# IRFM/librir

Hardware: NVIDIA B200
Metric: frames/s at 640x512 u16 (full per-frame pipeline: bad-pixel correct + gaussian + translate + pre-coder) (higher is better)
Workload: dtype u16

## Files before the change

include/librir_b200.h:

```cpp
#ifndef LIBRIR_B200_H
#define LIBRIR_B200_H

#include <stddef.h>
#include <stdint.h>

#ifdef __cplusplus
extern "C" {
#endif

#define RIRB_API __attribute__((visibility("default")))


RIRB_API int translate(int type, void* src, void* dst, int w, int h, float dx, float dy, void* background,
                       const char* strategy);

RIRB_API int gaussian_filter(float* src, float* dst, int w, int h, float sigma);

RIRB_API int find_median_pixel(unsigned short* pixels, int size, float percent);
RIRB_API int find_median_pixel_mask(unsigned short* pixels, unsigned char* mask, int size, float percent);

RIRB_API int bad_pixels_create(unsigned short* first_image, int width, int height);
RIRB_API int bad_pixels_correct(int handle, unsigned short* in, unsigned short* out);
RIRB_API void bad_pixels_destroy(int handle);

// ... 59 lines not shown
RIRB_API int rirb_decode_movie(const unsigned char* lo, const unsigned char* hi, long long nframes, int w, int h, int gop,
                               int delta, long long first_frame, unsigned short* movie);
RIRB_API int rirb_key_frames(long long nframes, int gop, unsigned char* key);

RIRB_API int rirb_lossy_open(int w, int h, int stop_lossy_height, int low_error, int high_error, double std_factor,
                             int running_average, int subtract_min, int remove_bad_pixels);
RIRB_API int rirb_lossy_add_images(int handle, const unsigned short* frames, long long nframes, unsigned short* out, int* errors);
RIRB_API int rirb_lossy_set_parameter(int handle, const char* key, const char* value);
RIRB_API void rirb_lossy_close(int handle);
RIRB_API int rirb_lossy_get_min(int handle, int* min_value);

RIRB_API int rirb_process_movie_host(int handle, const unsigned short* frames, long long nframes, int w, int h, float sigma,
                                     const float* dx, const float* dy, const char* strategy, unsigned int background, int gop,
                                     int delta, long long first_frame, unsigned char* lo, unsigned char* hi, float* smoothed);


RIRB_API int rirb_movie_stats(const unsigned short* pixels, size_t n, unsigned int* minmax, unsigned long long* hist,
                              int accumulate);
RIRB_API int rirb_hist_quantile(const unsigned long long* hist, long long count, float percent);
RIRB_API int rirb_get_background(const unsigned short* pixels, int size);


RIRB_API int rirb_attrs_open_file(const char* filename);
RIRB_API int rirb_attrs_open_from_memory(const void* ptr, long long size);
RIRB_API void rirb_attrs_close(int handle);
RIRB_API void rirb_attrs_discard(int handle);
RIRB_API void rirb_attrs_abandon(int handle);
RIRB_API int rirb_attrs_flush(int handle);
RIRB_API int rirb_attrs_image_count(int handle);
RIRB_API int rirb_attrs_global_attribute_count(int handle);
// ... 58 lines not shown
```

librir_b200/_lib.py:

```python
from __future__ import annotations

import ctypes as ct
import glob
import os

_HERE = os.path.dirname(os.path.abspath(__file__))
LIB_DIR = os.path.join(_HERE, "libs")


def lib_path() -> str:
    found = sorted(glob.glob(os.path.join(LIB_DIR, "*signal_processing*.so")))
    if not found:
        raise ImportError(
            "librir_b200: libs/libsignal_processing_b200.so is not built "
            "(run `python -c 'import __graft_entry__ as g; g.build()'` or `make -C librir_b200/csrc`)"
        )
    return found[0]


_vp, _i, _ll, _f, _sz = ct.c_void_p, ct.c_int, ct.c_longlong, ct.c_float, ct.c_size_t

SIGNATURES = {
    "translate": (_i, [_i, _vp, _vp, _i, _i, _f, _f, _vp, ct.c_char_p]),
    "gaussian_filter": (_i, [_vp, _vp, _i, _i, _f]),
# ... 29 lines not shown
    "rirb_split_yuv444": (_i, [_vp, _vp, _i, _i, _vp, _vp, _vp, _i, _i, _i]),
    "rirb_merge_yuv444": (_i, [_vp, _vp, _vp, _i, _i, _i, _i, _i, _vp, _vp]),
    "rirb_split_yuv420": (_i, [_vp, _vp, _i, _i, _vp, _i, _vp, _i]),
    "rirb_merge_yuv420": (_i, [_vp, _i, _vp, _i, _i, _i, _vp, _vp]),
    "rirb_precode_movie": (_i, [_vp, _ll, _i, _i, _i, _i, _ll, _vp, _vp]),
    "rirb_precode_movie_stats": (_i, [_vp, _ll, _i, _i, _i, _i, _ll, _vp, _vp, _vp, _vp, _i]),
    "rirb_decode_movie": (_i, [_vp, _vp, _ll, _i, _i, _i, _i, _ll, _vp]),
    "rirb_key_frames": (_i, [_ll, _i, _vp]),
    "rirb_lossy_open": (_i, [_i, _i, _i, _i, _i, ct.c_double, _i, _i, _i]),
    "rirb_lossy_add_images": (_i, [_i, _vp, _ll, _vp, _vp]),
    "rirb_lossy_close": (None, [_i]),
    "rirb_lossy_get_min": (_i, [_i, _vp]),
    "rirb_release_thread_resources": (None, []),
    "rirb_lossy_set_parameter": (_i, [_i, ct.c_char_p, ct.c_char_p]),
    "rirb_process_movie_host": (_i, [_i, _vp, _ll, _i, _i, _f, _vp, _vp, ct.c_char_p, ct.c_uint, _i, _i, _ll, _vp, _vp, _vp]),
    "rirb_movie_stats": (_i, [_vp, _sz, _vp, _vp, _i]),
    "rirb_hist_quantile": (_i, [_vp, _ll, _f]),
    "rirb_get_background": (_i, [_vp, _i]),
    "rirb_attrs_open_file": (_i, [ct.c_char_p]),
    "rirb_attrs_open_from_memory": (_i, [_vp, _ll]),
    "rirb_attrs_close": (None, [_i]),
    "rirb_attrs_discard": (None, [_i]),
    "rirb_attrs_abandon": (None, [_i]),
    "rirb_attrs_flush": (_i, [_i]),
    "rirb_attrs_image_count": (_i, [_i]),
    "rirb_attrs_global_attribute_count": (_i, [_i]),
    "rirb_attrs_global_attribute_name": (_i, [_i, _i, _vp, _vp]),
    "rirb_attrs_global_attribute_value": (_i, [_i, _i, _vp, _vp]),
    "rirb_attrs_frame_attribute_count": (_i, [_i, _i]),
    "rirb_attrs_frame_attribute_name": (_i, [_i, _i, _i, _vp, _vp]),
# ... 79 lines not shown
```

librir_b200/csrc/capi.cu:

```cuda
#include <dlfcn.h>
#include <math.h>
#include <stdarg.h>
#include <stdlib.h>
#include <string.h>

#include <map>
#include <memory>
#include <mutex>
#include <vector>

#include "../../include/librir_b200.h"
#include "common.cuh"
#include "kernels.h"

namespace rirb {

std::atomic<long long> g_launches{0};

struct ThreadState {
    char err[512] = {0};
    cudaStream_t stream = 0;
    static constexpr int SLOTS = 12;
    void* dev[SLOTS] = {};
    size_t cap[SLOTS] = {};
// ... 1482 lines not shown
        if (!ok(cudaMemcpyAsync(lo + a * fpx, d_lo, fpx * m, cudaMemcpyDefault, st), "download of the low-byte planes") ||
            !ok(cudaMemcpyAsync(hi + a * fpx, d_hi, fpx * m, cudaMemcpyDefault, st), "download of the high-byte planes") ||
            (smoothed && !ok(cudaMemcpyAsync(smoothed + a * fpx, d_sm, fpx * 4 * m, cudaMemcpyDefault, st), "download of the smoothed frames")))
            break;
    }
    for (int q = 0; q < HP_SLOTS; ++q) {
        cudaError_t e = cudaStreamSynchronize(hp.slot[q].stream);
        if (e != cudaSuccess && rc == 0) {
            set_error("process_movie_host: %s", cudaGetErrorString(e));
            rc = -1;
        }
    }
    return rc;
}

void rirb_release_thread_resources(void)
{
    if (tls.stream) (void)cudaStreamSynchronize(tls.stream);
    g_host_pipe.release();
    for (int d = 0; d < PIN_MAX_DEVICES; ++d) pin_rings[d].release();
    tls.release();
}

int rirb_movie_stats(const unsigned short* pixels, size_t n, unsigned int* minmax, unsigned long long* hist, int accumulate)
{
    if (!pixels || !minmax) {
        set_error("movie_stats: bad arguments");
        return -1;
    }
    RIRB_REQUIRE_DEVICE();
// ... 126 lines not shown
```

librir_b200/csrc/kernels.h:

```cpp
#pragma once
#include <cuda_runtime.h>
#include <stddef.h>

#include <initializer_list>

namespace rirb {

typedef unsigned short u16;
typedef unsigned char u8;

enum { STRAT_NOBORDER = 0, STRAT_BACKGROUND = 1, STRAT_WRAP = 2, STRAT_NEAREST = 3 };

int launch_hist_frame(const u16* img, size_t n, unsigned* hist65536, cudaStream_t st);
int launch_bp_detect(const u16* img, int w, int h, double std_factor, unsigned gthr, u8* mask, cudaStream_t st);
constexpr int BP_SPAN = 16384;
int launch_bp_correct(const u16* in, u16* out, const int* xy_dev, const int* span_off_dev, int w, int h, int clamp_value,
                      long long nframes, size_t frame_stride, cudaStream_t st);
int launch_bp_correct_inplace(u16* img, const int* xy_dev, int count, int w, int h, int clamp_value, long long nframes,
                              size_t frame_stride, cudaStream_t st);
int launch_loader_bp(u16* img, const int* xy_dev, const u8* mask, int count, int w, int h, long long nframes,
                     size_t frame_stride, cudaStream_t st);

int launch_loader_merge(const u8* lo, const u8* hi, u16* out, int w, int h, int hb, long long nframes, size_t frame_stride,
                        int min_t, int min_t_height, const int* xy_dev, const int* span_off_dev, const int* nbr_dev,
                        cudaStream_t st);

int launch_loader_add_min(u16* frames, int w, int t_rows, long long nframes, size_t frame_stride, int min_t, cudaStream_t st);
int launch_loader_fused(const u8* lo, const u8* hi, u16* out, int w, int h_full, int hb, long long nframes, int min_t, int t_rows,
                        const int* xy_dev, const int* nbr_dev, const int* row_off_dev, const u8* mask_dev, const float* dxs,
                        const float* dys, cudaStream_t st);

int launch_translate(int type, const void* src, void* dst, int w, int h, long long nframes, const float* dxs, const float* dys,
                     float dx0, float dy0, int strategy, const void* background_host, cudaStream_t st);
int launch_translate_u16(const u16* src, u16* dst, int w, int h, long long nframes, size_t src_stride, size_t dst_stride,
                         const float* dxs, const float* dys, float dx0, float dy0, int strategy, unsigned background, bool motion,
                         cudaStream_t st);

constexpr int GAUSS_MAX_RADIUS = 64;
struct GaussTaps {
    int radius;
    float k[2 * GAUSS_MAX_RADIUS + 1];
};
int gaussian_taps_host(float sigma, GaussTaps* taps);
int launch_gaussian_f32(const float* src, float* dst, int w, int h, long long nframes, const GaussTaps& taps, cudaStream_t st);
int launch_gaussian_u16(const u16* src, float* dst, int w, int h, long long nframes, const GaussTaps& taps, cudaStream_t st);
int launch_gaussian_u16_region(const u16* src, size_t src_row, size_t src_frame, float* dst, int w, int h, long long nframes,
                               const GaussTaps& taps, cudaStream_t st);
int launch_gaussian_f32_region(const float* src, size_t src_row, size_t src_frame, float* dst, int w, int h, long long nframes,
                               const GaussTaps& taps, cudaStream_t st);
int launch_gaussian_bp_u16(const u16* raw, u16* corrected, float* dst, int w, int h, long long nframes, const GaussTaps& taps,
                           const int* xy_dev, const int* row_off_dev, int clamp_value, cudaStream_t st);
// ... 44 lines not shown
inline int refuse_pageable(const char* what, std::initializer_list<Operand> ops)
{
    for (const Operand& o : ops)
        if (o.p && operand_memory_type(o.p) == cudaMemoryTypeUnregistered) {
            set_error("%s: %s is pageable host memory; pass device, managed or pinned memory", what, o.name);
            return -1;
        }
    return 0;
}

int launch_split_planes(const u16* img, const u8* it, int w, int h, u8* y_plane, u8* u_plane, u8* v_plane, int ls_y, int ls_u,
                        int ls_v, cudaStream_t st);
int launch_merge_planes(const u8* y_plane, const u8* u_plane, const u8* v_plane, int ls_y, int ls_u, int ls_v, int w, int h,
                        u16* img, u8* it, cudaStream_t st);
int launch_precode_movie(const u16* mov, long long nframes, int w, int h, int gop, int delta, long long first_frame, u8* lo,
                         u8* hi, cudaStream_t st);
int launch_precode_movie_stats(const u16* mov, long long nframes, int w, int h, int gop, int delta, long long first_frame, u8* lo,
                               u8* hi, unsigned* minmax, unsigned long long* hist, cudaStream_t st);
int launch_decode_movie(const u8* lo, const u8* hi, long long nframes, int w, int h, int gop, int delta, long long first_frame,
                        u16* mov, cudaStream_t st);

size_t zcoder_scratch_bytes(long long n, long long bytes_each, long long segment);
long long zcoder_frame_bound(long long bytes_each, long long segment);
int launch_zstd_encode(const u8* src, long long n, long long bytes_each, long long segment, u8* dst, long long dst_stride,
                       int rec_head, long long* sizes, long long** frame_offsets, void* scratch, cudaStream_t st);
size_t zcoder_lz_scratch_bytes(long long n, long long bytes_each, long long segment);
int launch_zstd_encode_lz(const u8* src, long long n, long long bytes_each, long long segment, u8* dst, long long dst_stride,
                          int rec_head, long long* sizes, long long** frame_offsets, void* scratch, cudaStream_t st);
size_t zdecoder_scratch_bytes(long long n, long long cap);
int zdecoder_frame_plain(const u8* f, long long size, long long cap);
int launch_zstd_decode(const u8* src, const long long* offsets, const unsigned* sizes, long long n, u8* dst, long long dst_stride,
                       long long cap, long long* status, void* scratch, cudaStream_t st);

// ... 23 lines not shown
```

librir_b200/csrc/precode.cu:

```cuda
#include "common.cuh"
#include "hist.cuh"
#include "kernels.h"

namespace rirb {

struct LoHi {
    uint4 lo, hi;
};

__device__ __forceinline__ LoHi split16(const U32x8& p)
{
    LoHi r;
    r.lo.x = __byte_perm(p.v[0], p.v[1], 0x6420);
    r.lo.y = __byte_perm(p.v[2], p.v[3], 0x6420);
    r.lo.z = __byte_perm(p.v[4], p.v[5], 0x6420);
    r.lo.w = __byte_perm(p.v[6], p.v[7], 0x6420);
    r.hi.x = __byte_perm(p.v[0], p.v[1], 0x7531);
    r.hi.y = __byte_perm(p.v[2], p.v[3], 0x7531);
    r.hi.z = __byte_perm(p.v[4], p.v[5], 0x7531);
    r.hi.w = __byte_perm(p.v[6], p.v[7], 0x7531);
    return r;
}

__device__ __forceinline__ U32x8 merge16(const uint4& lo, const uint4& hi)
// ... 73 lines not shown
__device__ __forceinline__ U32x8 sub16(const U32x8& a, const U32x8& b)
{
    U32x8 r;
#pragma unroll
    for (int i = 0; i < 8; ++i) r.v[i] = __vsub2(a.v[i], b.v[i]);
    return r;
}
__device__ __forceinline__ U32x8 add16(const U32x8& a, const U32x8& b)
{
    U32x8 r;
#pragma unroll
    for (int i = 0; i < 8; ++i) r.v[i] = __vadd2(a.v[i], b.v[i]);
    return r;
}

__global__ void __launch_bounds__(PC_THREADS)
delta_split_kernel(const u16* __restrict__ mov, u8* __restrict__ lo, u8* __restrict__ hi, size_t vec_per_frame, long long nframes,
                   int gop)
{
    const size_t i = (size_t)blockIdx.x * PC_THREADS + threadIdx.x;
    if (i >= vec_per_frame) return;
    const long long t0 = (long long)blockIdx.y * gop;
    const long long t1 = min(nframes, t0 + gop);
    U32x8 prev;
#pragma unroll
    for (int k = 0; k < 8; ++k) prev.v[k] = 0;
    for (long long t = t0; t < t1; t += PC_UNROLL) {
        U32x8 cur[PC_UNROLL];
#pragma unroll
        for (int k = 0; k < PC_UNROLL; ++k)
            if (t + k < t1) cur[k] = ld_stream256(mov + ((size_t)(t + k) * vec_per_frame + i) * 16);
#pragma unroll
        for (int k = 0; k < PC_UNROLL; ++k)
            if (t + k < t1) {
                LoHi r = split16(sub16(cur[k], prev));
                prev = cur[k];
                const size_t o = (size_t)(t + k) * vec_per_frame + i;
                st_stream(reinterpret_cast<uint4*>(lo) + o, r.lo);
                st_stream(reinterpret_cast<uint4*>(hi) + o, r.hi);
            }
    }
// ... 17 lines not shown
            if (t + k < t1) {
                const size_t o = (size_t)(t + k) * vec_per_frame + i;
                l[k] = ld_stream(reinterpret_cast<const uint4*>(lo) + o);
                h[k] = ld_stream(reinterpret_cast<const uint4*>(hi) + o);
            }
#pragma unroll
        for (int k = 0; k < PC_UNROLL; ++k)
            if (t + k < t1) {
                prev = add16(merge16(l[k], h[k]), prev);
                st_stream256(mov + ((size_t)(t + k) * vec_per_frame + i) * 16, prev);
            }
    }
}

__global__ void delta_split_scalar_kernel(const u16* __restrict__ mov, u8* __restrict__ lo, u8* __restrict__ hi, size_t npx,
                                          long long nframes, int gop)
{
    const size_t i = (size_t)blockIdx.x * blockDim.x + threadIdx.x;
    if (i >= npx) return;
    const long long t0 = (long long)blockIdx.y * gop;
    const long long t1 = min(nframes, t0 + gop);
    unsigned prev = 0;
    for (long long t = t0; t < t1; ++t) {
        unsigned cur = mov[(size_t)t * npx + i];
        unsigned r = (cur - prev) & 0xFFFFu;
        prev = cur;
        lo[(size_t)t * npx + i] = (u8)(r & 0xFF);
        hi[(size_t)t * npx + i] = (u8)(r >> 8);
    }
}
__global__ void delta_merge_scalar_kernel(const u8* __restrict__ lo, const u8* __restrict__ hi, u16* __restrict__ mov, size_t npx,
                                          long long nframes, int gop)
{
    const size_t i = (size_t)blockIdx.x * blockDim.x + threadIdx.x;
    if (i >= npx) return;
    const long long t0 = (long long)blockIdx.y * gop;
    const long long t1 = min(nframes, t0 + gop);
// ... 5 lines not shown
    }
}

constexpr long long MAX_GOPS_PER_LAUNCH = 65535;

static bool movie_vectorizable(const void* mov, const void* lo, const void* hi, size_t npx)
{
    return (npx % 16 == 0) && aligned32(mov) && aligned16(lo) && aligned16(hi);
}

constexpr int PS_THREADS = 1024;

template <bool DELTA>
__global__ void __launch_bounds__(PS_THREADS, 1)
split_stats_kernel(const u16* __restrict__ mov, u8* __restrict__ lo, u8* __restrict__ hi, size_t vec_per_frame, long long nframes,
                   int gop, unsigned* __restrict__ minmax, unsigned long long* __restrict__ hist)
{
    extern __shared__ unsigned sh[];
    for (unsigned i = threadIdx.x; i < HIST_SMEM_BINS; i += PS_THREADS) sh[i] = 0;
    __syncthreads();
    const long long ngop = (nframes + gop - 1) / gop;
    const long long blocks = (long long)((vec_per_frame + PS_THREADS - 1) / PS_THREADS);
    unsigned lo2 = 0xFFFFFFFFu, hi2 = 0u;
    for (long long item = blockIdx.x; item < blocks * ngop; item += gridDim.x) {
        const long long g = item / blocks;
        const size_t i = (size_t)(item - g * blocks) * PS_THREADS + threadIdx.x;
        if (i >= vec_per_frame) continue;
        const long long t0 = g * gop, t1 = min(nframes, t0 + gop);
        U32x8 prev;
#pragma unroll
        for (int k = 0; k < 8; ++k) prev.v[k] = 0;
        for (long long t = t0; t < t1; t += PC_UNROLL) {
            U32x8 cur[PC_UNROLL];
#pragma unroll
            for (int k = 0; k < PC_UNROLL; ++k)
                if (t + k < t1) cur[k] = ld_stream256(mov + ((size_t)(t + k) * vec_per_frame + i) * 16);
#pragma unroll
            for (int k = 0; k < PC_UNROLL; ++k)
                if (t + k < t1) {
                    const LoHi r = split16(DELTA ? sub16(cur[k], prev) : cur[k]);
                    if (DELTA) prev = cur[k];
                    const size_t o = (size_t)(t + k) * vec_per_frame + i;
                    st_stream(reinterpret_cast<uint4*>(lo) + o, r.lo);
                    st_stream(reinterpret_cast<uint4*>(hi) + o, r.hi);
#pragma unroll
                    for (int q = 0; q < 8; ++q) {
                        const unsigned w2 = cur[k].v[q];
                        lo2 = __vminu2(lo2, w2);
                        hi2 = __vmaxu2(hi2, w2);
                        count_px(w2 & 0xFFFFu, sh, hist);
                        count_px(w2 >> 16, sh, hist);
                    }
                }
        }
    }
    hist_flush(min(lo2 & 0xFFFFu, lo2 >> 16), max(hi2 & 0xFFFFu, hi2 >> 16), sh, minmax, hist, true);
}

int launch_precode_movie_stats(const u16* mov, long long nframes, int w, int h, int gop, int delta, long long first_frame, u8* lo,
                               u8* hi, unsigned* minmax, unsigned long long* hist, cudaStream_t st)
{
    if (nframes <= 0 || w <= 0 || h <= 0) return 0;
    const size_t npx = (size_t)w * h;
    if (gop < 1) gop = 1;
    if (!movie_vectorizable(mov, lo, hi, npx) || !hist || !minmax) return 1;
    if (delta && first_frame % gop != 0) {
        set_error("precode: with delta on, a shard must start on a key frame (first_frame %lld, GOP %d)", first_frame, gop);
        return -1;
    }
    const size_t vpf = npx / 16;
    const size_t smem = HIST_SMEM_BINS * sizeof(unsigned);
    const long long items = ceil_div((long long)vpf, PS_THREADS) * ceil_div(nframes, gop);
    const unsigned grid = (unsigned)min((long long)sm_count(), items);
    if (delta) {
        RIRB_SMEM_ATTR(split_stats_kernel<true>, smem);
        RIRB_LAUNCH(split_stats_kernel<true>, grid, PS_THREADS, smem, st, mov, lo, hi, vpf, nframes, gop, minmax, hist);
    } else {
        RIRB_SMEM_ATTR(split_stats_kernel<false>, smem);
        RIRB_LAUNCH(split_stats_kernel<false>, grid, PS_THREADS, smem, st, mov, lo, hi, vpf, nframes, gop, minmax, hist);
    }
    return 0;
}

int launch_precode_movie(const u16* mov, long long nframes, int w, int h, int gop, int delta, long long first_frame, u8* lo,
                         u8* hi, cudaStream_t st)
{
    if (nframes <= 0 || w <= 0 || h <= 0) return 0;
    const size_t npx = (size_t)w * h;
    if (gop < 1) gop = 1;
    if (!delta) {
        const size_t n = npx * (size_t)nframes;
        size_t done = 0;
        if (aligned32(mov) && aligned16(lo) && aligned16(hi) && n >= 16) {
            const size_t nvec = n / 16;
            RIRB_LAUNCH(split_flat_kernel, (unsigned)ceil_div((long long)nvec, PC_THREADS * PC_UNROLL), PC_THREADS, 0, st, mov, lo,
                        hi, nvec);
            done = nvec * 16;
        }
        if (done < n)
            RIRB_LAUNCH(split_scalar_kernel, (unsigned)ceil_div((long long)(n - done), 256), 256, 0, st, mov, lo, hi, done, n);
        return 0;
    }
    if (first_frame % gop != 0) {
        set_error("precode: with delta on, a shard must start on a key frame (first_frame %lld, GOP %d)", first_frame, gop);
        return -1;
    }
    const bool vec = movie_vectorizable(mov, lo, hi, npx);
    const long long span = (long long)MAX_GOPS_PER_LAUNCH * gop;
    for (long long f0 = 0; f0 < nframes; f0 += span) {
        const long long n = min(nframes - f0, span);
        const size_t off = (size_t)f0 * npx;
        const unsigned ngop = (unsigned)ceil_div(n, gop);
        if (vec) {
            const size_t vpf = npx / 16;
            dim3 grid((unsigned)ceil_div((long long)vpf, PC_THREADS), ngop);
            RIRB_LAUNCH(delta_split_kernel, grid, PC_THREADS, 0, st, mov + off, lo + off, hi + off, vpf, n, gop);
        } else {
            dim3 grid((unsigned)ceil_div((long long)npx, 256), ngop);
            RIRB_LAUNCH(delta_split_scalar_kernel, grid, 256, 0, st, mov + off, lo + off, hi + off, npx, n, gop);
        }
    }
    return 0;
}

int launch_decode_movie(const u8* lo, const u8* hi, long long nframes, int w, int h, int gop, int delta, long long first_frame,
                        u16* mov, cudaStream_t st)
{
    if (nframes <= 0 || w <= 0 || h <= 0) return 0;
    const size_t npx = (size_t)w * h;
    if (gop < 1) gop = 1;
    if (!delta) {
        const size_t n = npx * (size_t)nframes;
        size_t done = 0;
        if (aligned32(mov) && aligned16(lo) && aligned16(hi) && n >= 16) {
// ... 75 lines not shown
```

librir_b200/csrc/translate.cu:

```cuda
#include <stdlib.h>

#include "common.cuh"
#include "kernels.h"
#include "sort9.cuh"
#include "tma.cuh"

namespace rirb {

template <typename T> struct Pix {
    __device__ static __forceinline__ double to_double(T v) { return (double)v; }
    __device__ static __forceinline__ T from_double(double v) { return (T)v; }
};
struct BoolPix {
    u8 v;
};
template <> struct Pix<BoolPix> {
    __device__ static __forceinline__ double to_double(BoolPix b) { return b.v ? 1.0 : 0.0; }
    __device__ static __forceinline__ BoolPix from_double(double v) { return BoolPix{(u8)(v != 0.0)}; }
};

__device__ __forceinline__ unsigned long long f2size(float v) { return (unsigned long long)(long long)v; }
__device__ __forceinline__ unsigned long long wrap_idx(unsigned long long v, unsigned long long n) { return (v + n) % n; }

__device__ __forceinline__ double blend4(double p1, double p2, double p3, double p4, double u, double v)
// ... 711 lines not shown
        unpack9<XOFF>(lds128(srow), lds128(srow + 16), pb);
        if (clamp_rt) pb[8] = pb[7];
        unsigned A, B;
        asm volatile("ld.shared.v2.u32 {%0,%1}, [%2];" : "=r"(A), "=r"(B) : "r"(rab + k * (int)sizeof(RowAB)));
        if (B != ROW_SLOW) blend_rows<XOFF, MOTION>(pb, pt, A, B, ca, cb, magic, orow);
        orow += w;
#pragma unroll
        for (int j = 0; j < 9; ++j) pt[j] = pb[j];
    }
}

template <bool MOTION>
__global__ void __launch_bounds__(TW_THREADS, 5)
translate_u16_rows_kernel(const __grid_constant__ CUtensorMap tmap, const u16* __restrict__ src, u16* __restrict__ dst, int w, int h,
                          size_t src_stride, size_t dst_stride, const float* __restrict__ dxs, const float* __restrict__ dys,
                          float dx0, float dy0, int strategy, unsigned background, int tiles_y, const int* __restrict__ order)
{
    extern __shared__ __align__(128) unsigned char smem_raw[];
    __shared__ __align__(8) unsigned long long bar[TT_STAGES];
    __shared__ __align__(8) RowAB rowab[3][TT_H];
    __shared__ unsigned done[TT_STAGES];
    __shared__ EdgeTable edge_tab[2];
    const int f = order ? order[blockIdx.y] : (int)blockIdx.y;
    const int x0t = blockIdx.x * TT_W;
    const float dx = dxs ? dxs[f] : dx0;
    const float dy = dys ? dys[f] : dy0;
    const float fw = (float)w;
    const float fh = (float)h;
    const int sx = (int)fminf(fmaxf(floorf(-dx), -fw - 16.f), fw + 16.f);
    const int sy = (int)fminf(fmaxf(floorf(-dy), -fh - 16.f), fh + 16.f);
    const int xs = (x0t + sx) & ~15;
    const int xoff = (x0t + sx) - xs;
// ... 32 lines not shown
        const int l = (int)px;
        const int rt = (int)(px + 1.0f);
        const float un = tap_u(px, x);
        const bool cl = ok && (rt == w) && (l == w - 1) && (l == x + sx);
        ok = ok && (un >= 0.f) && (cl || rt == l + 1);
        edge_tab[e].wt[i] = make_hweights(ok ? un : 0.f);
        const unsigned vb = __ballot_sync(0x0000FFFFu, ok), cb2 = __ballot_sync(0x0000FFFFu, cl);
        const unsigned ob = __ballot_sync(0x0000FFFFu, (px < 0) || !(px < fw)), lb = __ballot_sync(0x0000FFFFu, px < 0);
        if (i == 0) {
            edge_tab[e].valid = (vb >> (8 * e)) & 0xFFu;
            edge_tab[e].clamped = (cb2 >> (8 * e)) & 0xFFu;
            edge_tab[e].outside = (ob >> (8 * e)) & 0xFFu;
            edge_tab[e].below = (lb >> (8 * e)) & 0xFFu;
        }
    }
    if (warp < 3 && warp < tiles_y) make_table(warp);
    __syncthreads();
    if (warp < TT_STAGES && warp < tiles_y) issue_box(warp, warp);

    const int cx = lane & 15, half = lane >> 4;
    const int r0 = 2 * TW_ROWS * warp + TW_ROWS * half;
    const int x0 = x0t + 8 * cx;
    const int isplit = (8 - xoff) & 7;
    const float pxf = (float)x0 - dx, pxl = (float)(x0 + 7) - dx;
    const float u0 = tap_u(pxf, x0), u7 = tap_u(pxl, x0 + 7);
    bool xfast = (x0 + 8 <= w) && !(pxf < 0) && (pxl < fw) && (u0 >= 0.f) && (u7 >= 0.f) && ((int)(pxl + 1.0f) == (int)pxl + 1);
    if (isplit == 0) {
        xfast = xfast && (u0 == u7);
    } else {
        const float pxa = (float)(x0 + isplit - 1) - dx, pxb = (float)(x0 + isplit) - dx;
        xfast = xfast && (tap_u(pxa, x0 + isplit - 1) == u0) && (tap_u(pxb, x0 + isplit) == u7) && ((int)(pxa + 1.0f) == (int)pxa + 1);
    }
    const bool clamp_rt = (x0 + sx + 8 == w);
    const HWeights ca = make_hweights(u0), cb = make_hweights(u7);
    const unsigned slowcols = __ballot_sync(0xFFFFFFFFu, !xfast && x0 < w) & 0xFFFFu;
    const u16* frame = src + (size_t)f * src_stride;
    u16* oframe = dst + (size_t)f * dst_stride;

#pragma unroll 1
    for (int ty = 0; ty < tiles_y; ++ty) {
        const int stage = ty % TT_STAGES;
        const int tslot = ty % 3;
        const unsigned parity = (unsigned)(ty / TT_STAGES) & 1u;
        const int y0t = ty * TT_H, ys = y0t + sy;
        mbar_wait(&bar[stage], parity);
        const u16* tile = reinterpret_cast<const u16*>(smem_raw + stage * TT_STAGE_BYTES);
        if (xfast) {
            const uint32_t srow = smem_addr(tile + r0 * TT_BW + 8 * cx + (xoff & 8));
            const uint32_t rab = smem_addr(&rowab[tslot][r0]);
            u16* orow = oframe + (size_t)(y0t + r0) * w + x0;
            switch (xoff & 7) {
            case 0: fast_column<0, MOTION>(srow, rab, clamp_rt, ca, cb, orow, (size_t)w); break;
            case 1: fast_column<1, MOTION>(srow, rab, clamp_rt, ca, cb, orow, (size_t)w); break;
            case 2: fast_column<2, MOTION>(srow, rab, clamp_rt, ca, cb, orow, (size_t)w); break;
            case 3: fast_column<3, MOTION>(srow, rab, clamp_rt, ca, cb, orow, (size_t)w); break;
            case 4: fast_column<4, MOTION>(srow, rab, clamp_rt, ca, cb, orow, (size_t)w); break;
            case 5: fast_column<5, MOTION>(srow, rab, clamp_rt, ca, cb, orow, (size_t)w); break;
            case 6: fast_column<6, MOTION>(srow, rab, clamp_rt, ca, cb, orow, (size_t)w); break;
// ... 97 lines not shown
                }
#pragma unroll 1
                for (int c = lane; c < TT_W; c += 32)
                    if (!((generic_cols >> (c >> 3)) & 1u)) slow_pixel(c, wr0 + rr);
            }
        }
        __syncwarp();
        unsigned last = 0;
        if (lane == 0) {
            unsigned old;
            asm volatile("atom.acq_rel.cta.shared.add.u32 %0, [%1], 1;" : "=r"(old) : "r"(smem_addr(&done[stage])) : "memory");
            last = (old == TW_WARPS - 1);
        }
        last = __shfl_sync(0xFFFFFFFFu, last, 0);
        if (last) {
            if (ty + TT_STAGES < tiles_y) issue_box(stage, ty + TT_STAGES);
            if (ty + 3 < tiles_y) make_table(ty + 3);
        }
    }
}

__global__ void __launch_bounds__(1024) translate_order_kernel(const float* __restrict__ dxs, int n, int w, int* __restrict__ order)
{
    __shared__ int count[8], start[8];
    const float fw = (float)w;
    if (threadIdx.x < 8) count[threadIdx.x] = 0;
    __syncthreads();
    auto key = [&](int f) { return (int)fminf(fmaxf(floorf(-dxs[f]), -fw - 16.f), fw + 16.f) & 7; };
    for (int f = threadIdx.x; f < n; f += blockDim.x) atomicAdd(&count[key(f)], 1);
    __syncthreads();
    if (threadIdx.x == 0) {
        int a = 0;
        for (int k = 0; k < 8; ++k) {
            start[k] = a;
            a += count[k];
        }
    }
    __syncthreads();
    for (int f = threadIdx.x; f < n; f += blockDim.x) order[atomicAdd(&start[key(f)], 1)] = f;
}

int launch_translate_u16(const u16* src, u16* dst, int w, int h, long long nframes, size_t src_stride, size_t dst_stride,
                         const float* dxs, const float* dys, float dx0, float dy0, int strategy, unsigned background, bool motion,
                         cudaStream_t st)
{
    if (nframes <= 0 || w <= 0 || h <= 0) return 0;
    const bool tma_enabled = option_enabled(OPT_TRANSLATE_TMA);
    const int tiles_x = (int)ceil_div(w, TT_W), tiles_y = (int)ceil_div(h, TT_H);
    if (tma_enabled && (w % 8 == 0) && aligned16(dst) && (dst_stride % 8 == 0) && tma_compatible(src, (size_t)w * 2, src_stride * 2)) {
        const size_t smem = (size_t)TT_STAGES * TT_STAGE_BYTES;
        RIRB_SMEM_ATTR((translate_u16_tma_kernel<true, false>), smem);
        RIRB_SMEM_ATTR((translate_u16_tma_kernel<false, false>), smem);
        RIRB_SMEM_ATTR((translate_u16_rows_kernel<true>), smem);
        RIRB_SMEM_ATTR((translate_u16_rows_kernel<false>), smem);
        for (long long f0 = 0; f0 < nframes; f0 += 65535) {
            const long long n = min(nframes - f0, 65535LL);
            const u16* s0 = src + f0 * src_stride;
            u16* d0 = dst + f0 * dst_stride;
            const float* dx_p = dxs ? dxs + f0 : nullptr;
            const float* dy_p = dys ? dys + f0 : nullptr;
            CUtensorMap tmap;
            if (make_movie_tensor_map(&tmap, s0, 2, w, h, n, (size_t)w * 2, src_stride * 2, TT_BW, TT_BH) != 0) return -1;
            const dim3 tgrid((unsigned)tiles_x, (unsigned)n);
            const PlaneSrc none{};
            if (option_enabled(OPT_TRANSLATE_ROWS)) {
                int* order = nullptr;
                if ((motion || option_value(OPT_TRANSLATE_ROWS) >= 2) && dx_p && n > 1) {
                    order = (int*)scratch_buffer(8, sizeof(int) * 65536);
                    if (!order) return -1;
                    RIRB_LAUNCH(translate_order_kernel, 1, 1024, 0, st, dx_p, (int)n, w, order);
                }
                if (motion)
                    RIRB_LAUNCH((translate_u16_rows_kernel<true>), tgrid, TW_THREADS, smem, st, tmap, s0, d0, w, h, src_stride, dst_stride,
                                dx_p, dy_p, dx0, dy0, strategy, background, tiles_y, order);
                else
                    RIRB_LAUNCH((translate_u16_rows_kernel<false>), tgrid, TW_THREADS, smem, st, tmap, s0, d0, w, h, src_stride, dst_stride,
                                dx_p, dy_p, dx0, dy0, strategy, background, tiles_y, order);
                continue;
            }
            if (motion)
                RIRB_LAUNCH((translate_u16_tma_kernel<true, false>), tgrid, TT_THREADS, smem, st, tmap, tmap, s0, d0, w, h, src_stride,
                            dst_stride, dx_p, dy_p, dx0, dy0, strategy, background, tiles_y, none);
            else
                RIRB_LAUNCH((translate_u16_tma_kernel<false, false>), tgrid, TT_THREADS, smem, st, tmap, tmap, s0, d0, w, h, src_stride,
                            dst_stride, dx_p, dy_p, dx0, dy0, strategy, background, tiles_y, none);
        }
        return 0;
    }
    dim3 block(32, 8);
    dim3 grid((unsigned)ceil_div(ceil_div(w, TR_PX), 32), (unsigned)ceil_div(h, 8), (unsigned)min(nframes, 32768LL));
    if (motion)
        RIRB_LAUNCH(translate_u16_kernel<true>, grid, block, 0, st, src, dst, w, h, nframes, src_stride, dst_stride, dxs, dys, dx0,
// ... 66 lines not shown
```

librir_b200/movie.py:

```python
from __future__ import annotations

import ctypes as ct
from dataclasses import dataclass

import numpy as np

from . import _lib
from . import signal_processing as sp
from . import video_io as vio


@dataclass(frozen=True)
class FrameShard:
    rank: int
    world: int
    start: int
    stop: int

    @property
    def nframes(self) -> int:
        return self.stop - self.start


def shard_frames(nframes: int, world: int, rank: int, gop: int = vio.DEFAULT_GOP) -> FrameShard:
# ... 65 lines not shown

    def histogram(self) -> np.ndarray:
        return self.hist.cpu().numpy().astype(np.uint64)

    def quantile(self, percent: float = 0.5) -> int:
        lib = _lib.load()
        _lib.use_torch_stream()
        r = lib.rirb_hist_quantile(ct.c_void_p(self.hist.data_ptr()), self.count, float(percent))
        return _lib.check(r, "hist_quantile")

    def background(self) -> int:
        h4 = self.hist.view(16384, 4).sum(dim=1)
        return (int(h4.argmax().item()) << 2) + 1


@dataclass
class PipelineConfig:
    width: int = 640
    height: int = 512
    sigma: float = 1.0
    strategy: str = "nearest"
    gop: int = vio.DEFAULT_GOP
    delta: bool = True
    chunk_frames: int = 4096
    fuse_stats: bool = True


class FramePipeline:

    def __init__(self, cfg: PipelineConfig, device="cuda"):
        import torch

        self.cfg = cfg
        self.device = torch.device(device)
        n, h, w = cfg.chunk_frames, cfg.height, cfg.width
        self.corrected = torch.empty((n, h, w), dtype=torch.uint16, device=self.device)
        self.smoothed = torch.empty((n, h, w), dtype=torch.float32, device=self.device)
        self.registered = torch.empty((n, h, w), dtype=torch.uint16, device=self.device)
        self.lo = torch.empty((n, h, w), dtype=torch.uint8, device=self.device)
        self.hi = torch.empty((n, h, w), dtype=torch.uint8, device=self.device)
# ... 6 lines not shown
    @property
    def STAGES(self):
        if self.cfg.fuse_stats:
            return ("bp_correct", "gaussian_u16_f32", "translate_u16", "precode_delta_split_stats")
        return ("bp_correct", "gaussian_u16_f32", "translate_u16", "precode_delta_split", "stats_minmax_hist")

    def process_chunk(self, frames, dx, dy, first_frame: int, with_stats: bool = True, events=None):
        import torch

        if self.bad_pixels is None:
            raise RuntimeError("FramePipeline: call set_first_frame() first")
        n = frames.shape[0]
        c, s, r = self.corrected[:n], self.smoothed[:n], self.registered[:n]
        lo, hi = self.lo[:n], self.hi[:n]
        mark = (lambda i: events[i].record(torch.cuda.current_stream())) if events is not None else (lambda i: None)
        mark(0)
        self.bad_pixels.correct_batch(frames, out=c)
        mark(1)
        sp.gaussian_filter_batch(c, self.cfg.sigma, out=s)
        mark(2)
        sp.translate_batch(c, dx, dy, self.cfg.strategy, background=0, out=r)
        mark(3)
        if self.cfg.fuse_stats:
            vio.precode_movie(r, self.cfg.gop, self.cfg.delta, first_frame, out=(lo, hi), stats=self.stats if with_stats else None)
            mark(4)
        else:
            vio.precode_movie(r, self.cfg.gop, self.cfg.delta, first_frame, out=(lo, hi))
            mark(4)
            if with_stats:
                self.stats.update(r)
            mark(5)
        return c, s, r, lo, hi

    def process_host(self, frames_host, dx_host, dy_host, first_frame: int, lo_host, hi_host, sub_frames: int = 256,
                     slots: int = 3):
        import torch

        if self.bad_pixels is None:
            raise RuntimeError("FramePipeline: call set_first_frame() first")
        n = frames_host.shape[0]
        gop = self.cfg.gop
        sub = max(gop, sub_frames // gop * gop) if self.cfg.delta else sub_frames
        ns = len(self._e2e) if hasattr(self, "_e2e") else slots
        if ns * sub > self.cfg.chunk_frames:
            raise RuntimeError(f"process_host: {ns} slots of {sub} frames do not fit the {self.cfg.chunk_frames}-frame chunk buffers; "
                               "lower sub_frames or slots, or raise chunk_frames")
        if not hasattr(self, "_e2e"):
# ... 84 lines not shown
```

Measured before the change: 1.070 million.

## Add single-call chunk pipeline with optional L2-sized frame blocking

Adds rirb_process_chunk, a C entry point that runs bad-pixel correction, gaussian, translate and precode+stats in one call and optionally in frame blocks sized to fit L2. When blocking is on, the translate and precode kernels split work into sub-GOP pieces or tile-row segments so small blocks still fill the GPU, and delta coding then reads the previous frame across piece boundaries. The Python fused path now calls this entry point, replacing four separate ctypes calls and their per-call Python overhead. The default block size is 0, which means one block covering the whole chunk, so the main change by default is lower host overhead. The blocking path adds extra launches and sub-GOP splitting.

```diff
diff --git a/include/librir_b200.h b/include/librir_b200.h
--- a/include/librir_b200.h
+++ b/include/librir_b200.h
@@ -97,6 +97,12 @@
                                      const float* dx, const float* dy, const char* strategy, unsigned int background, int gop,
                                      int delta, long long first_frame, unsigned char* lo, unsigned char* hi, float* smoothed);
 
+RIRB_API int rirb_process_chunk(int handle, const unsigned short* frames, long long nframes, int w, int h, float sigma,
+                                const float* dx, const float* dy, const char* strategy, unsigned int background, int gop,
+                                int delta, long long first_frame, unsigned short* corrected, float* smoothed,
+                                unsigned short* registered, unsigned char* lo, unsigned char* hi, unsigned int* minmax,
+                                unsigned long long* hist, int accumulate, long long block_frames, void* const* stage_events);
+
 
 RIRB_API int rirb_movie_stats(const unsigned short* pixels, size_t n, unsigned int* minmax, unsigned long long* hist,
                               int accumulate);
diff --git a/librir_b200/_lib.py b/librir_b200/_lib.py
--- a/librir_b200/_lib.py
+++ b/librir_b200/_lib.py
@@ -67,6 +67,8 @@
     "rirb_release_thread_resources": (None, []),
     "rirb_lossy_set_parameter": (_i, [_i, ct.c_char_p, ct.c_char_p]),
     "rirb_process_movie_host": (_i, [_i, _vp, _ll, _i, _i, _f, _vp, _vp, ct.c_char_p, ct.c_uint, _i, _i, _ll, _vp, _vp, _vp]),
+    "rirb_process_chunk": (_i, [_i, _vp, _ll, _i, _i, _f, _vp, _vp, ct.c_char_p, ct.c_uint, _i, _i, _ll, _vp, _vp, _vp, _vp,
+                                _vp, _vp, _vp, _i, _ll, _vp]),
     "rirb_movie_stats": (_i, [_vp, _sz, _vp, _vp, _i]),
     "rirb_hist_quantile": (_i, [_vp, _ll, _f]),
     "rirb_get_background": (_i, [_vp, _i]),
diff --git a/librir_b200/csrc/capi.cu b/librir_b200/csrc/capi.cu
--- a/librir_b200/csrc/capi.cu
+++ b/librir_b200/csrc/capi.cu
@@ -1520,6 +1520,71 @@
     return rc;
 }
 
+int rirb_process_chunk(int handle, const unsigned short* frames, long long nframes, int w, int h, float sigma, const float* dx,
+                       const float* dy, const char* strategy, unsigned int background, int gop, int delta, long long first_frame,
+                       unsigned short* corrected, float* smoothed, unsigned short* registered, unsigned char* lo, unsigned char* hi,
+                       unsigned int* minmax, unsigned long long* hist, int accumulate, long long block_frames,
+                       void* const* stage_events)
+{
+    auto s = find_handle_here(handle, "process_chunk");
+    if (!s) return -1;
+    const int strat = strategy_code(strategy);
+    if (!frames || !dx || !dy || !corrected || !smoothed || !registered || !lo || !hi || (!minmax != !hist) || w != s->w ||
+        h != s->h || nframes < 0 || gop < 1 || strat < 0 || strat == STRAT_NOBORDER || block_frames < 0 ||
+        (delta && first_frame % gop != 0)) {
+        set_error("process_chunk: bad arguments");
+        return -1;
+    }
+    if (nframes == 0) return 0;
+    GaussTaps taps;
+    if (gaussian_taps_host(sigma, &taps) != 0) return -1;
+    RIRB_REQUIRE_DEVICE();
+    const size_t fpx = (size_t)w * h, n = fpx * (size_t)nframes;
+    const Operand ops[] = {{"frames", frames, n * 2}, {"dx", dx, 4 * (size_t)nframes}, {"dy", dy, 4 * (size_t)nframes},
+                           {"corrected", corrected, n * 2}, {"smoothed", smoothed, n * 4}, {"registered", registered, n * 2},
+                           {"lo", lo, n}, {"hi", hi, n}, {"minmax", minmax, 2 * sizeof(unsigned)},
+                           {"hist", hist, 65536 * sizeof(unsigned long long)}};
+    for (const Operand& o : ops)
+        if (o.p && !operand_on_device(o.p)) {
+            set_error("process_chunk: %s is not device memory", o.name);
+            return -1;
+        }
+    if (refuse_overlap("process_chunk", {ops[0], ops[1], ops[2]}, {ops[3], ops[4], ops[5], ops[6], ops[7], ops[8], ops[9]})) return -1;
+    cudaStream_t st = tls.stream;
+    if (minmax && !accumulate && launch_stats_init(minmax, hist, st) != 0) return -1;
+    const long long B = block_frames == 0 ? nframes : block_frames;
+    const bool blocked = B < nframes;
+    for (long long b0 = 0; b0 < nframes; b0 += B) {
+        const long long m = nframes - b0 < B ? nframes - b0 : B;
+        const bool last = b0 + m == nframes;
+        const size_t o = (size_t)b0 * fpx;
+        const int phase = delta ? (int)(b0 % gop) : 0;
+#define RIRB_MARK(i) \
+    if (last && stage_events) RIRB_CUDA_OK(cudaEventRecord((cudaEvent_t)stage_events[i], st))
+        if (launch_bp_correct(frames + o, corrected + o, s->xy_dev, s->span_off_dev, w, h, s->clamp_value, m, fpx, st) != 0) return -1;
+        RIRB_MARK(0);
+        if (launch_gaussian_u16(corrected + o, smoothed + o, w, h, m, taps, st) != 0) return -1;
+        RIRB_MARK(1);
+        if (launch_translate_u16(corrected + o, registered + o, w, h, m, fpx, fpx, dx + b0, dy + b0, 0.f, 0.f, strat,
+                                 background & 0xFFFFu, false, st, blocked) != 0)
+            return -1;
+        RIRB_MARK(2);
+        int rc = 1;
+        if (minmax) {
+            rc = launch_precode_movie_stats(registered + o, m, w, h, gop, delta, first_frame, lo + o, hi + o, minmax, hist, st, phase,
+                                            blocked);
+            if (rc < 0) return -1;
+        }
+        if (rc == 1) {
+            if (launch_precode_movie(registered + o, m, w, h, gop, delta, first_frame, lo + o, hi + o, st, phase, blocked) != 0) return -1;
+            if (minmax && launch_movie_stats(registered + o, fpx * (size_t)m, nullptr, minmax, hist, st) != 0) return -1;
+        }
+        RIRB_MARK(3);
+#undef RIRB_MARK
+    }
+    return 0;
+}
+
 void rirb_release_thread_resources(void)
 {
     if (tls.stream) (void)cudaStreamSynchronize(tls.stream);
diff --git a/librir_b200/csrc/kernels.h b/librir_b200/csrc/kernels.h
--- a/librir_b200/csrc/kernels.h
+++ b/librir_b200/csrc/kernels.h
@@ -34,7 +34,7 @@
                      float dx0, float dy0, int strategy, const void* background_host, cudaStream_t st);
 int launch_translate_u16(const u16* src, u16* dst, int w, int h, long long nframes, size_t src_stride, size_t dst_stride,
                          const float* dxs, const float* dys, float dx0, float dy0, int strategy, unsigned background, bool motion,
-                         cudaStream_t st);
+                         cudaStream_t st, bool fill = false);
 
 constexpr int GAUSS_MAX_RADIUS = 64;
 struct GaussTaps {
@@ -109,9 +109,10 @@
 int launch_merge_planes(const u8* y_plane, const u8* u_plane, const u8* v_plane, int ls_y, int ls_u, int ls_v, int w, int h,
                         u16* img, u8* it, cudaStream_t st);
 int launch_precode_movie(const u16* mov, long long nframes, int w, int h, int gop, int delta, long long first_frame, u8* lo,
-                         u8* hi, cudaStream_t st);
+                         u8* hi, cudaStream_t st, int phase = 0, bool fill = false);
 int launch_precode_movie_stats(const u16* mov, long long nframes, int w, int h, int gop, int delta, long long first_frame, u8* lo,
-                               u8* hi, unsigned* minmax, unsigned long long* hist, cudaStream_t st);
+                               u8* hi, unsigned* minmax, unsigned long long* hist, cudaStream_t st, int phase = 0,
+                               bool fill = false);
 int launch_decode_movie(const u8* lo, const u8* hi, long long nframes, int w, int h, int gop, int delta, long long first_frame,
                         u16* mov, cudaStream_t st);
 
diff --git a/librir_b200/csrc/precode.cu b/librir_b200/csrc/precode.cu
--- a/librir_b200/csrc/precode.cu
+++ b/librir_b200/csrc/precode.cu
@@ -111,17 +111,42 @@
     return r;
 }
 
+__host__ __device__ __forceinline__ long long piece_index(long long u, int gop, int seg)
+{
+    return (u / gop) * ((gop + seg - 1) / seg) + (u % gop) / seg;
+}
+__host__ __device__ __forceinline__ long long piece_count(long long n, int gop, int seg, int phase)
+{
+    return piece_index(phase + n - 1, gop, seg) - piece_index(phase, gop, seg) + 1;
+}
+struct Piece {
+    long long t0, t1;
+    bool key;
+};
+__device__ __forceinline__ Piece piece_of(long long p, long long n, int gop, int seg, int phase)
+{
+    const long long per = (gop + seg - 1) / seg;
+    p += piece_index(phase, gop, seg);
+    const long long g = p / per, u0 = g * gop + (p - g * per) * seg, u1 = min(u0 + seg, g * gop + gop);
+    Piece r;
+    r.t0 = max(u0, (long long)phase) - phase;
+    r.t1 = min(u1, (long long)phase + n) - phase;
+    r.key = (r.t0 + phase) % gop == 0;
+    return r;
+}
+
 __global__ void __launch_bounds__(PC_THREADS)
 delta_split_kernel(const u16* __restrict__ mov, u8* __restrict__ lo, u8* __restrict__ hi, size_t vec_per_frame, long long nframes,
-                   int gop)
+                   int gop, int seg, int phase)
 {
     const size_t i = (size_t)blockIdx.x * PC_THREADS + threadIdx.x;
     if (i >= vec_per_frame) return;
-    const long long t0 = (long long)blockIdx.y * gop;
-    const long long t1 = min(nframes, t0 + gop);
+    const Piece pc = piece_of(blockIdx.y, nframes, gop, seg, phase);
+    const long long t0 = pc.t0, t1 = pc.t1;
     U32x8 prev;
 #pragma unroll
     for (int k = 0; k < 8; ++k) prev.v[k] = 0;
+    if (!pc.key) prev = ld_stream256(mov + ((size_t)(t0 - 1) * vec_per_frame + i) * 16);
     for (long long t = t0; t < t1; t += PC_UNROLL) {
         U32x8 cur[PC_UNROLL];
 #pragma unroll
@@ -169,13 +194,13 @@
 }
 
 __global__ void delta_split_scalar_kernel(const u16* __restrict__ mov, u8* __restrict__ lo, u8* __restrict__ hi, size_t npx,
-                                          long long nframes, int gop)
+                                          long long nframes, int gop, int seg, int phase)
 {
     const size_t i = (size_t)blockIdx.x * blockDim.x + threadIdx.x;
     if (i >= npx) return;
-    const long long t0 = (long long)blockIdx.y * gop;
-    const long long t1 = min(nframes, t0 + gop);
-    unsigned prev = 0;
+    const Piece pc = piece_of(blockIdx.y, nframes, gop, seg, phase);
+    const long long t0 = pc.t0, t1 = pc.t1;
+    unsigned prev = pc.key ? 0u : (unsigned)mov[(size_t)(t0 - 1) * npx + i];
     for (long long t = t0; t < t1; ++t) {
         unsigned cur = mov[(size_t)t * npx + i];
         unsigned r = (cur - prev) & 0xFFFFu;
@@ -211,23 +236,25 @@
 template <bool DELTA>
 __global__ void __launch_bounds__(PS_THREADS, 1)
 split_stats_kernel(const u16* __restrict__ mov, u8* __restrict__ lo, u8* __restrict__ hi, size_t vec_per_frame, long long nframes,
-                   int gop, unsigned* __restrict__ minmax, unsigned long long* __restrict__ hist)
+                   int gop, int seg, int phase, unsigned* __restrict__ minmax, unsigned long long* __restrict__ hist)
 {
     extern __shared__ unsigned sh[];
     for (unsigned i = threadIdx.x; i < HIST_SMEM_BINS; i += PS_THREADS) sh[i] = 0;
     __syncthreads();
-    const long long ngop = (nframes + gop - 1) / gop;
+    const long long npieces = piece_count(nframes, gop, seg, phase);
     const long long blocks = (long long)((vec_per_frame + PS_THREADS - 1) / PS_THREADS);
     unsigned lo2 = 0xFFFFFFFFu, hi2 = 0u;
-    for (long long item = blockIdx.x; item < blocks * ngop; item += gridDim.x) {
+    for (long long item = blockIdx.x; item < blocks * npieces; item += gridDim.x) {
         const long long g = item / blocks;
         const size_t i = (size_t)(item - g * blocks) * PS_THREADS + threadIdx.x;
         if (i >= vec_per_frame) continue;
-        const long long t0 = g * gop, t1 = min(nframes, t0 + gop);
+        const Piece pc = piece_of(g, nframes, gop, seg, phase);
+        const long long t1 = pc.t1;
         U32x8 prev;
 #pragma unroll
         for (int k = 0; k < 8; ++k) prev.v[k] = 0;
-        for (long long t = t0; t < t1; t += PC_UNROLL) {
+        if (DELTA && !pc.key) prev = ld_stream256(mov + ((size_t)(pc.t0 - 1) * vec_per_frame + i) * 16);
+        for (long long t = pc.t0; t < t1; t += PC_UNROLL) {
             U32x8 cur[PC_UNROLL];
 #pragma unroll
             for (int k = 0; k < PC_UNROLL; ++k)
@@ -254,8 +281,15 @@
     hist_flush(min(lo2 & 0xFFFFu, lo2 >> 16), max(hi2 & 0xFFFFu, hi2 >> 16), sh, minmax, hist, true);
 }
 
+static int piece_length(long long nframes, int gop, long long blocks, long long target)
+{
+    if (ceil_div(nframes, gop) * blocks >= target) return gop;
+    const long long s = nframes * blocks / target;
+    return (int)(s < 1 ? 1 : (s > gop ? gop : s));
+}
+
 int launch_precode_movie_stats(const u16* mov, long long nframes, int w, int h, int gop, int delta, long long first_frame, u8* lo,
-                               u8* hi, unsigned* minmax, unsigned long long* hist, cudaStream_t st)
+                               u8* hi, unsigned* minmax, unsigned long long* hist, cudaStream_t st, int phase, bool fill)
 {
     if (nframes <= 0 || w <= 0 || h <= 0) return 0;
     const size_t npx = (size_t)w * h;
@@ -265,22 +299,25 @@
         set_error("precode: with delta on, a shard must start on a key frame (first_frame %lld, GOP %d)", first_frame, gop);
         return -1;
     }
+    if (!delta) phase = 0;
     const size_t vpf = npx / 16;
     const size_t smem = HIST_SMEM_BINS * sizeof(unsigned);
-    const long long items = ceil_div((long long)vpf, PS_THREADS) * ceil_div(nframes, gop);
+    const long long blocks = ceil_div((long long)vpf, PS_THREADS);
+    const int seg = fill ? piece_length(nframes + phase, gop, blocks, 2LL * sm_count()) : gop;
+    const long long items = blocks * piece_count(nframes, gop, seg, phase);
     const unsigned grid = (unsigned)min((long long)sm_count(), items);
     if (delta) {
         RIRB_SMEM_ATTR(split_stats_kernel<true>, smem);
-        RIRB_LAUNCH(split_stats_kernel<true>, grid, PS_THREADS, smem, st, mov, lo, hi, vpf, nframes, gop, minmax, hist);
+        RIRB_LAUNCH(split_stats_kernel<true>, grid, PS_THREADS, smem, st, mov, lo, hi, vpf, nframes, gop, seg, phase, minmax, hist);
     } else {
         RIRB_SMEM_ATTR(split_stats_kernel<false>, smem);
-        RIRB_LAUNCH(split_stats_kernel<false>, grid, PS_THREADS, smem, st, mov, lo, hi, vpf, nframes, gop, minmax, hist);
+        RIRB_LAUNCH(split_stats_kernel<false>, grid, PS_THREADS, smem, st, mov, lo, hi, vpf, nframes, gop, seg, phase, minmax, hist);
     }
     return 0;
 }
 
 int launch_precode_movie(const u16* mov, long long nframes, int w, int h, int gop, int delta, long long first_frame, u8* lo,
-                         u8* hi, cudaStream_t st)
+                         u8* hi, cudaStream_t st, int phase, bool fill)
 {
     if (nframes <= 0 || w <= 0 || h <= 0) return 0;
     const size_t npx = (size_t)w * h;
@@ -303,18 +340,21 @@
         return -1;
     }
     const bool vec = movie_vectorizable(mov, lo, hi, npx);
+    const long long xblocks = vec ? ceil_div((long long)(npx / 16), PC_THREADS) : ceil_div((long long)npx, 256);
+    const int seg = fill ? piece_length(nframes + phase, gop, xblocks, 8LL * sm_count()) : gop;
     const long long span = (long long)MAX_GOPS_PER_LAUNCH * gop;
     for (long long f0 = 0; f0 < nframes; f0 += span) {
         const long long n = min(nframes - f0, span);
         const size_t off = (size_t)f0 * npx;
-        const unsigned ngop = (unsigned)ceil_div(n, gop);
+        const int ph = (int)((phase + f0) % gop);
+        const unsigned np = (unsigned)piece_count(n, gop, seg, ph);
         if (vec) {
             const size_t vpf = npx / 16;
-            dim3 grid((unsigned)ceil_div((long long)vpf, PC_THREADS), ngop);
-            RIRB_LAUNCH(delta_split_kernel, grid, PC_THREADS, 0, st, mov + off, lo + off, hi + off, vpf, n, gop);
+            dim3 grid((unsigned)xblocks, np);
+            RIRB_LAUNCH(delta_split_kernel, grid, PC_THREADS, 0, st, mov + off, lo + off, hi + off, vpf, n, gop, seg, ph);
         } else {
-            dim3 grid((unsigned)ceil_div((long long)npx, 256), ngop);
-            RIRB_LAUNCH(delta_split_scalar_kernel, grid, 256, 0, st, mov + off, lo + off, hi + off, npx, n, gop);
+            dim3 grid((unsigned)xblocks, np);
+            RIRB_LAUNCH(delta_split_scalar_kernel, grid, 256, 0, st, mov + off, lo + off, hi + off, npx, n, gop, seg, ph);
         }
     }
     return 0;
diff --git a/librir_b200/csrc/translate.cu b/librir_b200/csrc/translate.cu
--- a/librir_b200/csrc/translate.cu
+++ b/librir_b200/csrc/translate.cu
@@ -749,8 +749,10 @@
 __global__ void __launch_bounds__(TW_THREADS, 5)
 translate_u16_rows_kernel(const __grid_constant__ CUtensorMap tmap, const u16* __restrict__ src, u16* __restrict__ dst, int w, int h,
                           size_t src_stride, size_t dst_stride, const float* __restrict__ dxs, const float* __restrict__ dys,
-                          float dx0, float dy0, int strategy, unsigned background, int tiles_y, const int* __restrict__ order)
-{
+                          float dx0, float dy0, int strategy, unsigned background, int tiles_y, int seg_tiles,
+                          const int* __restrict__ order)
+{
+    const int ty_begin = blockIdx.z * seg_tiles, ty_end = min(tiles_y, ty_begin + seg_tiles);
     extern __shared__ __align__(128) unsigned char smem_raw[];
     __shared__ __align__(8) unsigned long long bar[TT_STAGES];
     __shared__ __align__(8) RowAB rowab[3][TT_H];
@@ -813,9 +815,9 @@
             edge_tab[e].below = (lb >> (8 * e)) & 0xFFu;
         }
     }
-    if (warp < 3 && warp < tiles_y) make_table(warp);
+    if (warp < 3 && ty_begin + warp < ty_end) make_table(ty_begin + warp);
     __syncthreads();
-    if (warp < TT_STAGES && warp < tiles_y) issue_box(warp, warp);
+    if (warp < TT_STAGES && ty_begin + warp < ty_end) issue_box(warp, ty_begin + warp);
 
     const int cx = lane & 15, half = lane >> 4;
     const int r0 = 2 * TW_ROWS * warp + TW_ROWS * half;
@@ -837,10 +839,10 @@
     u16* oframe = dst + (size_t)f * dst_stride;
 
 #pragma unroll 1
-    for (int ty = 0; ty < tiles_y; ++ty) {
-        const int stage = ty % TT_STAGES;
+    for (int ty = ty_begin; ty < ty_end; ++ty) {
+        const int stage = (ty - ty_begin) % TT_STAGES;
         const int tslot = ty % 3;
-        const unsigned parity = (unsigned)(ty / TT_STAGES) & 1u;
+        const unsigned parity = (unsigned)((ty - ty_begin) / TT_STAGES) & 1u;
         const int y0t = ty * TT_H, ys = y0t + sy;
         mbar_wait(&bar[stage], parity);
         const u16* tile = reinterpret_cast<const u16*>(smem_raw + stage * TT_STAGE_BYTES);
@@ -968,8 +970,8 @@
         }
         last = __shfl_sync(0xFFFFFFFFu, last, 0);
         if (last) {
-            if (ty + TT_STAGES < tiles_y) issue_box(stage, ty + TT_STAGES);
-            if (ty + 3 < tiles_y) make_table(ty + 3);
+            if (ty + TT_STAGES < ty_end) issue_box(stage, ty + TT_STAGES);
+            if (ty + 3 < ty_end) make_table(ty + 3);
         }
     }
 }
@@ -996,7 +998,7 @@
 
 int launch_translate_u16(const u16* src, u16* dst, int w, int h, long long nframes, size_t src_stride, size_t dst_stride,
                          const float* dxs, const float* dys, float dx0, float dy0, int strategy, unsigned background, bool motion,
-                         cudaStream_t st)
+                         cudaStream_t st, bool fill)
 {
     if (nframes <= 0 || w <= 0 || h <= 0) return 0;
     const bool tma_enabled = option_enabled(OPT_TRANSLATE_TMA);
@@ -1018,6 +1020,10 @@
             const dim3 tgrid((unsigned)tiles_x, (unsigned)n);
             const PlaneSrc none{};
             if (option_enabled(OPT_TRANSLATE_ROWS)) {
+                const long long want = 4LL * 5 * sm_count();
+                int seg = tiles_y;
+                if (fill && n * tiles_x < want) seg = (int)ceil_div(tiles_y, min((long long)tiles_y, ceil_div(want, n * tiles_x)));
+                const dim3 rgrid((unsigned)tiles_x, (unsigned)n, (unsigned)ceil_div(tiles_y, seg));
                 int* order = nullptr;
                 if ((motion || option_value(OPT_TRANSLATE_ROWS) >= 2) && dx_p && n > 1) {
                     order = (int*)scratch_buffer(8, sizeof(int) * 65536);
@@ -1025,11 +1031,11 @@
                     RIRB_LAUNCH(translate_order_kernel, 1, 1024, 0, st, dx_p, (int)n, w, order);
                 }
                 if (motion)
-                    RIRB_LAUNCH((translate_u16_rows_kernel<true>), tgrid, TW_THREADS, smem, st, tmap, s0, d0, w, h, src_stride, dst_stride,
-                                dx_p, dy_p, dx0, dy0, strategy, background, tiles_y, order);
+                    RIRB_LAUNCH((translate_u16_rows_kernel<true>), rgrid, TW_THREADS, smem, st, tmap, s0, d0, w, h, src_stride, dst_stride,
+                                dx_p, dy_p, dx0, dy0, strategy, background, tiles_y, seg, order);
                 else
-                    RIRB_LAUNCH((translate_u16_rows_kernel<false>), tgrid, TW_THREADS, smem, st, tmap, s0, d0, w, h, src_stride, dst_stride,
-                                dx_p, dy_p, dx0, dy0, strategy, background, tiles_y, order);
+                    RIRB_LAUNCH((translate_u16_rows_kernel<false>), rgrid, TW_THREADS, smem, st, tmap, s0, d0, w, h, src_stride, dst_stride,
+                                dx_p, dy_p, dx0, dy0, strategy, background, tiles_y, seg, order);
                 continue;
             }
             if (motion)
diff --git a/librir_b200/movie.py b/librir_b200/movie.py
--- a/librir_b200/movie.py
+++ b/librir_b200/movie.py
@@ -1,7 +1,8 @@
 from __future__ import annotations
 
 import ctypes as ct
-from dataclasses import dataclass
+import os
+from dataclasses import dataclass, field
 
 import numpy as np
 
@@ -103,6 +104,8 @@
         return (int(h4.argmax().item()) << 2) + 1
 
 
+DEFAULT_L2_BLOCK_BYTES = 0
+
 @dataclass
 class PipelineConfig:
     width: int = 640
@@ -113,6 +116,12 @@
     delta: bool = True
     chunk_frames: int = 4096
     fuse_stats: bool = True
+    l2_block_bytes: int = field(default_factory=lambda: int(os.environ.get("RIRB_L2_BLOCK_BYTES", DEFAULT_L2_BLOCK_BYTES)))
+
+    def block_frames(self) -> int:
+        if self.l2_block_bytes <= 0:
+            return 0
+        return max(1, self.l2_block_bytes // (4 * self.width * self.height))
 
 
 class FramePipeline:
@@ -149,6 +158,9 @@
         c, s, r = self.corrected[:n], self.smoothed[:n], self.registered[:n]
         lo, hi = self.lo[:n], self.hi[:n]
         mark = (lambda i: events[i].record(torch.cuda.current_stream())) if events is not None else (lambda i: None)
+        if self.cfg.fuse_stats:
+            self._run_chunk(frames, dx, dy, first_frame, with_stats, events)
+            return c, s, r, lo, hi
         mark(0)
         self.bad_pixels.correct_batch(frames, out=c)
         mark(1)
@@ -156,16 +168,61 @@
         mark(2)
         sp.translate_batch(c, dx, dy, self.cfg.strategy, background=0, out=r)
         mark(3)
-        if self.cfg.fuse_stats:
-            vio.precode_movie(r, self.cfg.gop, self.cfg.delta, first_frame, out=(lo, hi), stats=self.stats if with_stats else None)
-            mark(4)
-        else:
-            vio.precode_movie(r, self.cfg.gop, self.cfg.delta, first_frame, out=(lo, hi))
-            mark(4)
-            if with_stats:
-                self.stats.update(r)
-            mark(5)
+        vio.precode_movie(r, self.cfg.gop, self.cfg.delta, first_frame, out=(lo, hi))
+        mark(4)
+        if with_stats:
+            self.stats.update(r)
+        mark(5)
         return c, s, r, lo, hi
+
+    def _run_chunk(self, frames, dx, dy, first_frame, with_stats, events):
+        import torch
+
+        lib = _lib.load()
+        what = "process_chunk"
+        sp._prepare_device_call(frames)
+        frames = sp._operand(frames, what, "frames", dtype=np.uint16)
+        n, h, w = frames.shape
+        if (h, w) != (self.cfg.height, self.cfg.width) or n > self.cfg.chunk_frames:
+            raise RuntimeError(f"{what}: frames of shape {tuple(frames.shape)} do not fit the pipeline's "
+                               f"{self.cfg.chunk_frames} x {self.cfg.height} x {self.cfg.width} buffers")
+        dx, dy = (self._shifts(v, n, name) for v, name in ((dx, "dx"), (dy, "dy")))
+        stream = torch.cuda.current_stream()
+        stage_events = None
+        if events is not None:
+            events[0].record(stream)
+            for e in events[1:5]:
+                e.record(stream)
+            stage_events = (ct.c_void_p * 4)(*[e.cuda_event for e in events[1:5]])
+        st = self.stats if with_stats else None
+        if st is not None and st._fresh:
+            st._sums[65536] = 0
+        p = sp._ptr
+        r = lib.rirb_process_chunk(self.bad_pixels.handle, p(frames), n, w, h, float(self.cfg.sigma), p(dx), p(dy),
+                                   sp.toCharP(self.cfg.strategy), 0, int(self.cfg.gop), int(bool(self.cfg.delta)),
+                                   int(first_frame), p(self.corrected), p(self.smoothed), p(self.registered), p(self.lo),
+                                   p(self.hi), ct.c_void_p(st.minmax.data_ptr()) if st is not None else None,
+                                   ct.c_void_p(st.hist.data_ptr()) if st is not None else None,
+                                   0 if st is None or st._fresh else 1, self.cfg.block_frames(), stage_events)
+        _lib.check(r, what)
+        if st is not None:
+            st._fresh = False
+            st._sums[65536] += n * h * w
+
+    def _shifts(self, v, n, name):
+        import torch
+
+        if sp._is_torch(v) and v.numel() == n and n != 1:
+            return sp._operand(v.reshape(n) if v.is_contiguous() else v, "process_chunk", name, (n,), np.float32)
+        if sp._is_torch(v) or np.ndim(v) == 0 or np.size(v) == 1:
+            t = torch.as_tensor(v, dtype=torch.float32, device=self.device).reshape(-1)
+            if t.numel() != 1:
+                raise RuntimeError(f"process_chunk: {name} has {t.numel()} shifts for {n} frames")
+            return t.expand(n).contiguous()
+        a = np.ascontiguousarray(v, dtype=np.float32)
+        if a.shape != (n,):
+            raise RuntimeError(f"process_chunk: {name} has {a.size} shifts for {n} frames")
+        return torch.from_numpy(a).to(self.device)
 
     def process_host(self, frames_host, dx_host, dy_host, first_frame: int, lo_host, hi_host, sub_frames: int = 256,
                      slots: int = 3):
```

Result: no change. 1.063 million, median of 6 (-0.7%).
